# trukanduk/pq_huffman

Measured on AMD Instinct MI355X. Metric: Mvec/s encode+decode round-trip, 128-d fp32 M=8 K=256; % HBM-read roofline, higher is better.
Workload: dtype f32

## Files before the change

### include/pqh.h

```cpp
#ifndef _PQH_H
#define _PQH_H

#include <stddef.h>
#include <stdint.h>

#include "fast_nn_block.h"
#include "huffman.h"

#ifdef __cplusplus
extern "C" {
#endif

typedef enum {
    PQH_OK = 0,
    PQH_ERR_ARG = -1,
    PQH_ERR_NO_DEVICE = -2,
    PQH_ERR_HIP = -3,
    PQH_ERR_UNSUPPORTED = -4,
    PQH_ERR_CODE_TOO_LONG = -5,
    PQH_ERR_CORRUPT = -6,
    PQH_ERR_NOMEM = -7,
    PQH_ERR_CAPACITY = -8,
    PQH_ERR_REMOTE = -9,
    PQH_ERR_COMM = -10
} pqh_status_t;

typedef struct pqh_ctx pqh_ctx_t;

int pqh_ctx_create(pqh_ctx_t** ctx, int device);
int pqh_ctx_create_cu_limited(pqh_ctx_t** ctx, int device, int cus);
int pqh_ctx_create_cu_split(pqh_ctx_t** ctx, int device, int cus, int complement);
void* pqh_ctx_stream(const pqh_ctx_t* ctx);
int pqh_ctx_destroy(pqh_ctx_t* ctx);
int pqh_ctx_release_scratch(pqh_ctx_t* ctx);
int pqh_ctx_set_stream(pqh_ctx_t* ctx, void* hip_stream);
int pqh_ctx_sync(pqh_ctx_t* ctx);
enum { PQH_TUNE_ASSIGN_WGS_PER_CU = 1, PQH_TUNE_HIST_SPLIT = 2, PQH_TUNE_HIST_BLOCK = 3,
       PQH_TUNE_ENC_IMPL = 4, PQH_TUNE_SEARCH_GROUPS = 5 };
int pqh_ctx_set_tuning(pqh_ctx_t* ctx, int key, double value);
const char* pqh_status_string(int status);
const char* pqh_ctx_last_error(const pqh_ctx_t* ctx);
int pqh_device_count(int* count);

typedef struct pqh_pq pqh_pq_t;

int pqh_pq_create(pqh_ctx_t* ctx, const float* centroids, int m, int k, int dsub, pqh_pq_t** pq);
int pqh_pq_destroy(pqh_pq_t* pq);

int pqh_pq_assign(pqh_ctx_t* ctx, const pqh_pq_t* pq, const float* d_x, long long n,
                  long long ld_x, void* d_codes, uint32_t* d_counts, int mode);
int pqh_pq_assign_parts(pqh_ctx_t* ctx, const pqh_pq_t* pq, const float* d_x, long long n,
                        long long ld_x, void* d_codes, long long ld_codes, uint32_t* d_counts,
                        int mode);
int pqh_pq_last_rerank_count(pqh_ctx_t* ctx, unsigned long long* count);

int pqh_pq_error(pqh_ctx_t* ctx, const pqh_pq_t* pq, const float* d_x, long long n,
                 long long ld_x, const void* d_codes, double* error_out);
int pqh_pq_reconstruct(pqh_ctx_t* ctx, const pqh_pq_t* pq, const void* d_codes, long long n,
                       float* d_out, long long ld_out);

int pqh_kmeans_train(pqh_ctx_t* ctx, const float* d_x, long long n, long long ld_x, int m,
                     int k, int dsub, int iters, float* centroids);

int pqh_histogram(pqh_ctx_t* ctx, const void* d_codes, long long n, int m, int k, int context,
                  const void* d_prev_row, uint32_t* d_counts);
int pqh_histogram_set(pqh_ctx_t* ctx, const void* d_codes, long long n, int m, int k,
                      int context, const void* d_prev_row, uint32_t* d_counts);
long long pqh_histogram_partial_bytes(long long n, int m, int k);
int pqh_histogram_parts(pqh_ctx_t* ctx, const void* d_codes, long long ld_codes, long long n,
                        int m, int k, int context, const void* d_prev_row, uint32_t* d_counts,
                        int set);
// ... 294 lines not shown
```

### pq_huffman_amd/codec.py

```python
from __future__ import annotations

import ctypes
import os
import tempfile
from dataclasses import dataclass

import numpy as np

from .capi import (EncodeOptions, HuffmanCodebook, PqhError, check, lib)

_libc = ctypes.CDLL(None)
_libc.fopen.restype = ctypes.c_void_p
_libc.fopen.argtypes = [ctypes.c_char_p, ctypes.c_char_p]
_libc.fclose.argtypes = [ctypes.c_void_p]
_libc.fwrite.argtypes = [ctypes.c_void_p, ctypes.c_size_t, ctypes.c_size_t, ctypes.c_void_p]
_libc.fseek.argtypes = [ctypes.c_void_p, ctypes.c_long, ctypes.c_int]


def _ptr(t):
    if t is None:
        return None
    if isinstance(t, np.ndarray):
        return t.ctypes.data_as(ctypes.c_void_p)
    return ctypes.c_void_p(t.data_ptr())
# ... 4 lines not shown
    return torch


def device_count() -> int:
    n = ctypes.c_int(0)
    lib().pqh_device_count(ctypes.byref(n))
    return n.value


class Context:

    def __init__(self, device: int = 0, stream=None, cus: int = 0, complement: bool = False):
        torch = _torch()
        self._deps = 0
        self._closing = False
        self.device = device
        torch.cuda.set_device(device)
        self.ptr = ctypes.c_void_p()
        if cus != 0:
            check(lib().pqh_ctx_create_cu_split(ctypes.byref(self.ptr), device, cus,
                                                int(complement)), "pqh_ctx_create_cu_split")
            self.stream = torch.cuda.ExternalStream(lib().pqh_ctx_stream(self.ptr), device=device)
            return
        self.stream = stream or torch.cuda.current_stream(device)
        check(lib().pqh_ctx_create(ctypes.byref(self.ptr), device), "pqh_ctx_create")
        check(lib().pqh_ctx_set_stream(self.ptr, ctypes.c_void_p(self.stream.cuda_stream)),
              "pqh_ctx_set_stream")

    def set_stream(self, stream) -> None:
        self.stream = stream
        check(lib().pqh_ctx_set_stream(self.ptr, ctypes.c_void_p(stream.cuda_stream)))

    TUNE = {"assign_wgs_per_cu": 1, "hist_split": 2, "hist_block": 3, "enc_impl": 4,
            "search_groups": 5}

    def set_tuning(self, **kw) -> "Context":
        for key, value in kw.items():
            check(lib().pqh_ctx_set_tuning(self.ptr, self.TUNE[key], float(value)),
                  f"pqh_ctx_set_tuning({key})")
        return self

    def sync(self) -> None:
        check(lib().pqh_ctx_sync(self.ptr), "pqh_ctx_sync")

    def release_scratch(self) -> None:
        check(lib().pqh_ctx_release_scratch(self.ptr), "pqh_ctx_release_scratch")

    def last_error(self) -> str:
        return (lib().pqh_ctx_last_error(self.ptr) or b"").decode()

    def _retain(self) -> None:
        self._deps += 1

    def _release(self) -> None:
        self._deps -= 1
        if self._closing and self._deps <= 0:
            self.close()

    def close(self) -> None:
        if self._deps > 0:
            self._closing = True
            return
        if self.ptr:
            lib().pqh_ctx_destroy(self.ptr)
            self.ptr = ctypes.c_void_p()

    def __del__(self):
# ... 939 lines not shown
```

### pq_huffman_amd/csrc/hip/pqh_assign.hip

```cpp
#include <algorithm>
#include <cmath>
#include <cstdlib>
#include <cstring>
#include <type_traits>
#include <vector>

#include "pqh_internal.h"

typedef __bf16 bf16x8 __attribute__((ext_vector_type(8)));
typedef float f32x16 __attribute__((ext_vector_type(16)));
typedef float f32x4 __attribute__((ext_vector_type(4)));

namespace {

#ifndef PQH_ASSIGN_WPG
#define PQH_ASSIGN_WPG 4
#endif
#ifndef PQH_ASSIGN_OCC_LARGE
#define PQH_ASSIGN_OCC_LARGE 2
#endif
#ifndef PQH_ASSIGN_RING
#define PQH_ASSIGN_RING 4
#endif
#ifndef PQH_ASSIGN_NB
// ... 1 lines not shown
#endif
#ifndef PQH_ASSIGN_OCC
#define PQH_ASSIGN_OCC (PQH_ASSIGN_NB == 1 ? 4 : 3)
#endif
#ifndef PQH_ASSIGN_DEFER
#define PQH_ASSIGN_DEFER 1
#endif
#ifndef PQH_ASSIGN_RQ
#define PQH_ASSIGN_RQ 128
#endif
#ifndef PQH_ASSIGN_RRMASK
#define PQH_ASSIGN_RRMASK 1
#endif
#ifndef PQH_ASSIGN_RRPAIR
#define PQH_ASSIGN_RRPAIR 1
#endif
#ifndef PQH_ASSIGN_RRPACK
#define PQH_ASSIGN_RRPACK 1
#endif
#ifndef PQH_ASSIGN_RRPICK
#define PQH_ASSIGN_RRPICK 1
#endif
#ifndef PQH_ASSIGN_RRSKIP
#define PQH_ASSIGN_RRSKIP 1
#endif
#ifndef PQH_ASSIGN_HANDOVER
#define PQH_ASSIGN_HANDOVER 1
#endif
#ifndef PQH_ASSIGN_EARLYX
#define PQH_ASSIGN_EARLYX 1
#endif
constexpr int kRqLds = PQH_ASSIGN_RQ;
constexpr int kWavesPerWG = PQH_ASSIGN_WPG;
constexpr int kNB = PQH_ASSIGN_NB;
#ifndef PQH_ASSIGN_CLDS
#define PQH_ASSIGN_CLDS 0
#endif
#ifndef PQH_ASSIGN_SHAREA
#define PQH_ASSIGN_SHAREA 0
#endif
constexpr int kAG = 8;
#ifndef PQH_ASSIGN_XAUX
#define PQH_ASSIGN_XAUX 0
#endif
constexpr bool kCentLds = PQH_ASSIGN_CLDS != 0;

template <int D>
struct Plan {
    static constexpr int MAIN = 2 * D;
    static constexpr int PM = (MAIN + 15) / 16;
    static constexpr int PL = (D + 15) / 16;
    static constexpr int PA = PM;
};

#ifndef PQH_ASSIGN_ASMMIN
#define PQH_ASSIGN_ASMMIN 0
#endif
#if PQH_ASSIGN_ASMMIN
__device__ __forceinline__ unsigned med3u(unsigned a, unsigned b, unsigned c) {
    unsigned r;
    asm("v_med3_f32 %0, %1, %2, %3" : "=v"(r) : "v"(a), "v"(b), "v"(c));
    return r;
}

__device__ __forceinline__ unsigned min3d(unsigned a, unsigned b, unsigned c, unsigned after) {
    unsigned r;
// ... 99 lines not shown
    return 0.0f;
}

template <int D>
__device__ __forceinline__ float exact_dist(const float* x, const float* c) {
#pragma clang fp contract(off)
    float acc = 0.0f;
#pragma unroll
    for (int j = 0; j < D; ++j) {
        float d = __fsub_rn(x[j], c[j]);
        acc = __fadd_rn(acc, __fmul_rn(d, d));
    }
    return acc;
}

constexpr int kStampWaves = 8192;
__device__ unsigned long long g_assign_stamps[kStampWaves][4];
__device__ unsigned long long g_assign_rr[kStampWaves][4];
#ifdef PQH_ASSIGN_STAMPS
#define PQH_RR_STAMP(var)                                                \
    do {                                                                 \
        asm volatile("s_waitcnt vmcnt(0) lgkmcnt(0)" ::: "memory");      \
        var = __builtin_amdgcn_s_memrealtime();                          \
    } while (0)
#endif

template <int D>
struct Slice {
    static constexpr bool HALF = D % 16 == 0;
    static constexpr int NP = HALF ? D / 16 : 1;
    static constexpr int XD = HALF ? D / 2 : D;
    static __device__ __forceinline__ int dim(int j, int h) {
        return HALF ? 16 * (j >> 3) + 8 * h + (j & 7) : j;
    }
};

__device__ __forceinline__ unsigned partner32(unsigned v) {
    const auto sw = __builtin_amdgcn_permlane32_swap(v, v, false, false);
    return (threadIdx.x & 32) ? sw[0] : sw[1];
}

template <int D>
__device__ __forceinline__ float norm_part(const float* xs) {
    float X = 0.0f;
#pragma unroll
    for (int j = 0; j < Slice<D>::XD; ++j) X = fmaf(xs[j], xs[j], X);
    return X;
}

template <int D>
__device__ __forceinline__ float norm_x(const float* xs) {
    float X = norm_part<D>(xs);
    if constexpr (Slice<D>::HALF) {
        const auto sw = __builtin_amdgcn_permlane32_swap(__float_as_uint(X), __float_as_uint(X),
                                                         false, false);
        X = __uint_as_float(sw[0]) + __uint_as_float(sw[1]);
    }
    return X;
}

template <int D>
__device__ __forceinline__ bool has_lo(const float* xs) {
    constexpr int XD = Slice<D>::XD;
    unsigned o = __float_as_uint(xs[0]);
    int j = 1;
    for (; j + 1 < XD; j += 2)
// ... 177 lines not shown
}

template <int D, int KT>
__device__ __forceinline__ f32x16 tile_scores(const uint4* src, const float* Cn, int lane, int t,
                                              const bf16x8* Bm, const bf16x8* Bl, bool lo_pass) {
    using P = Plan<D>;
    bf16x8 a[P::PA];
#pragma unroll
    for (int p = 0; p < P::PA; ++p) a[p] = frag_at<KT>(src, p, t, lane);
    return tile_scores_a<D>(a, Bm, Bl, lo_pass, tile_norms(Cn, t, lane >> 5));
}

__device__ __forceinline__ int tile_row(int t, int i, int h) {
    return 32 * t + (i & 3) + 8 * (i >> 2) + 4 * h;
}

__device__ __forceinline__ uint32_t score_mask(const f32x16& acc, float thr, uint32_t bits) {
#if PQH_ASSIGN_RRMASK && defined(__HIP_DEVICE_COMPILE__)
#pragma unroll
    for (int i = 15; i >= 0; --i) {
        const unsigned long long le = __ballot(acc[i] <= thr);
        asm("v_addc_co_u32_e64 %0, vcc, %0, %0, %1" : "+v"(bits) : "s"(le) : "vcc");
    }
    return bits;
#else
    uint32_t mk = 0;
#pragma unroll
    for (int i = 0; i < 16; ++i) mk |= (acc[i] <= thr ? 1u : 0u) << i;
    return (bits << 16) | mk;
#endif
}

template <int D, int KT, typename CodeT>
__global__ void __launch_bounds__(64 * kWavesPerWG, D == 32 ? 2 : KT > 8 ? PQH_ASSIGN_OCC_LARGE : PQH_ASSIGN_OCC)
pq_assign_mfma(const float* __restrict__ x, long long n, long long ldx, int m_total,
               const bf16x8* __restrict__ afrag, const float* __restrict__ cnorm,
               const float* __restrict__ cent,
               const float* __restrict__ cmax, const float* __restrict__ sqrt_cmax,
               CodeT* __restrict__ codes, uint32_t* __restrict__ counts,
               unsigned long long* __restrict__ rerank, uint32_t* __restrict__ sched, int gx,
               unsigned long long* __restrict__ rerank_next, uint32_t* __restrict__ sched_next,
               int prio, long long ldc) {
    using P = Plan<D>;
    constexpr int K = KT * 32;
    constexpr bool kLdsA = KT <= 8;
    constexpr int PB = KT <= 8 ? 4 : 8;
    constexpr unsigned PMASK = (1u << PB) - 1;
    static_assert(2 * KT <= (1 << PB), "P-group index must fit the key's low bits");
    extern __shared__ uint32_t hist_dyn[];
    auto hist = [&](int w) -> uint32_t* { return hist_dyn + w * K; };
    __shared__ uint4 As[kLdsA ? P::PA * KT * 64 : 1];
    __shared__ __attribute__((aligned(64))) float Cn[KT * 2 * 16];
    __shared__ uint2 rqs[kWavesPerWG][kRqLds];
    constexpr int kPairs = PQH_ASSIGN_HANDOVER && kWavesPerWG % 2 == 0 ? kWavesPerWG / 2 : 0;
    __shared__ uint32_t rq_box[kPairs ? kPairs : 1];
#ifndef PQH_ASSIGN_XLDS
#define PQH_ASSIGN_XLDS 1
#endif
    constexpr bool kXLds = PQH_ASSIGN_XLDS && KT <= 8 && Slice<D>::XD % 4 == 0;
    __shared__ __attribute__((aligned(16))) float xst[kXLds ? kWavesPerWG : 1][kXLds ? kNB : 1]
                                                     [kXLds ? Slice<D>::XD / 4 : 1][kXLds ? 256 : 1];
    __shared__ __attribute__((aligned(16))) float Cf[kLdsA && kCentLds ? K * D : 1];
    constexpr bool kShareA = !kLdsA && PQH_ASSIGN_SHAREA != 0;
    constexpr int kAR = 2 * kAG;
    __shared__ __attribute__((aligned(16))) uint4 Ar[kShareA ? kAR * P::PA * 64 : 1];

    const int lane = threadIdx.x & 63;
    const int wave = __builtin_amdgcn_readfirstlane(threadIdx.x >> 6);
    const int L = blockIdx.x;
    const bool inter = (gx & 7) == 0;
    const int m = inter ? (L >> 3) % m_total : L / gx;
    const int bx = inter ? (L / (8 * m_total)) * 8 + (L & 7) : L % gx;
    const int r = lane & 31;
    const int h = lane >> 5;
    pqh_set_prio(prio);
    if (L == 0 && wave == 0) {
        if (sched_next)
            for (int q = lane; q < kSchedMax * kXcds; q += 64)
                __hip_atomic_store(sched_next + q * kSchedStride, 0u, __ATOMIC_RELAXED,
                                   __HIP_MEMORY_SCOPE_AGENT);
        if (lane == 0)
            __hip_atomic_store(rerank_next, 0ull, __ATOMIC_RELAXED, __HIP_MEMORY_SCOPE_AGENT);
    }
    constexpr bool kEarlyX = PQH_ASSIGN_EARLYX != 0 && !kShareA;
    auto fill_lds = [&]() {
        const uint4* src = reinterpret_cast<const uint4*>(afrag) + (long long)m * P::PA * KT * 64;
        constexpr int kNA = P::PA * KT * 64, kThreads = 64 * kWavesPerWG;
        if constexpr (kLdsA && kEarlyX && kNA % kThreads == 0 && KT * 2 * 16 <= kThreads) {
            const int tid = (int)threadIdx.x;
            if (KT * 2 * 16 == kThreads || tid < KT * 2 * 16)
                Cn[tid] = cnorm[(long long)m * KT * 2 * 16 + tid];
#pragma unroll
            for (int j = 0; j < kNA / kThreads; ++j) As[tid + j * kThreads] = src[tid + j * kThreads];
        } else {
            if constexpr (kLdsA)
                for (int i = threadIdx.x; i < kNA; i += blockDim.x) As[i] = src[i];
            for (int i = threadIdx.x; i < KT * 2 * 16; i += blockDim.x)
                Cn[i] = cnorm[(long long)m * KT * 2 * 16 + i];
        }
        if (kLdsA && counts)
            for (int i = lane; i < K; i += 64) hist(wave)[i] = 0;
        if constexpr (kLdsA && kCentLds)
            for (int i = threadIdx.x; i < K * D; i += blockDim.x) Cf[i] = cent[(long long)m * K * D + i];
        if ((int)threadIdx.x < kPairs) rq_box[threadIdx.x] = 0u;
        __syncthreads();
    };
    if constexpr (!kEarlyX) fill_lds();
    const uint4* const asrc =
        kLdsA ? As : reinterpret_cast<const uint4*>(afrag) + (long long)m * P::PA * KT * 64;
    const auto arsrc = __builtin_amdgcn_make_buffer_rsrc(
        const_cast<uint4*>(reinterpret_cast<const uint4*>(afrag) + (long long)m * P::PA * KT * 64),
        0, P::PA * KT * 64 * 16, 0x00020000);
#ifdef PQH_ASSIGN_STAMPS
    const unsigned long long st0 = __builtin_amdgcn_s_memtime();
    const unsigned long long rt0 = __builtin_amdgcn_s_memrealtime();
    unsigned long long nbdone = 0, rr_ticks = 0, rr_batches = 0;
    unsigned long long rr_x = 0, rr_scr = 0, rr_cand = 0, rr_rounds = 0;
#endif
    const float cm = cmax[m];
    const float sc = sqrt_cmax[m];
    const TauCoef tq = tau_coef(cm, sc, sqrt_cmax[m_total + m]);
    const float ninf = opaque_ninf();
    const unsigned keymask = PB == 4 ? ~PMASK : opaque_u32(~PMASK);
    const float* cl = kLdsA && kCentLds ? Cf : cent + (long long)m * K * D;
    const int n32 = (int)n;
    const int nblk = (n32 + 31) / 32;
    const int nfull = n32 / 32;
    unsigned long long slow_count = 0;

    constexpr bool HALF = Slice<D>::HALF;
    constexpr int XD = Slice<D>::XD;
// ... 17 lines not shown
            const unsigned last = (unsigned)(left < 31 ? left : 31);
            off = __umul24(min((unsigned)r, last), ldx4) + xh_off;
        }
        const float* xp = reinterpret_cast<const float*>(xm + row0 * (long long)ldx4 + off);
        if constexpr (XD % 4 == 0) {
#pragma unroll
            for (int j = 0; j < XD; j += 4) {
                const f32x4 q = *reinterpret_cast<const f32x4*>(xp + (HALF ? 16 * (j >> 3) + (j & 7) : j));
                dst[j] = q.x; dst[j + 1] = q.y; dst[j + 2] = q.z; dst[j + 3] = q.w;
            }
        } else {
#pragma unroll
            for (int j = 0; j < XD; ++j) dst[j] = xp[j];
        }
    };
    auto load_x_lds = [&](int b, int slot) {
#ifdef PQH_ASSIGN_NOMEM
        b &= 63;
#endif
        long long row0 = (long long)b * 32;
        unsigned off = xlane_off;
        if (b >= nfull) {
            row0 = row0 < n - 1 ? row0 : n - 1;
            const long long left = n - 1 - row0;
            const unsigned last = (unsigned)(left < 31 ? left : 31);
            off = __umul24(min((unsigned)r, last), ldx4) + xh_off;
        }
        const float* xp = reinterpret_cast<const float*>(xm + row0 * (long long)ldx4 + off);
#pragma unroll
        for (int j = 0; j < XD; j += 4) {
#if defined(__HIP_DEVICE_COMPILE__)
            __builtin_amdgcn_global_load_lds(
                xp + (HALF ? 16 * (j >> 3) + (j & 7) : j),
                (__attribute__((address_space(3))) void*)(&xst[wave][slot][j / 4][0]), 16, 0,
                PQH_ASSIGN_XAUX);
#else
            (void)xp;
#endif
        }
    };
    auto read_x_lds = [&](int slot, float* dst) {
#pragma unroll
        for (int j = 0; j < XD; j += 4) {
            const f32x4 q = *reinterpret_cast<const f32x4*>(&xst[wave][slot][j / 4][lane * 4]);
            dst[j] = q.x; dst[j + 1] = q.y; dst[j + 2] = q.z; dst[j + 3] = q.w;
        }
    };
    auto read_ring = [&](int t, bf16x8* a) {
#pragma unroll
        for (int p = 0; p < P::PA; ++p)
            a[p] = *reinterpret_cast<const bf16x8*>(&Ar[((t % kAR) * P::PA + p) * 64 + lane]);
    };
    auto dma_group = [&](int g) {
        if constexpr (kShareA) {
            const uint4* src = reinterpret_cast<const uint4*>(afrag) + (long long)m * P::PA * KT * 64;
            static_assert((kAG * P::PA) % kWavesPerWG == 0, "whole pieces per wave");
#pragma unroll
            for (int i = 0; i < (kAG * P::PA) / kWavesPerWG; ++i) {
                const int q = wave + i * kWavesPerWG;
                const int t = g * kAG + q / P::PA, p = q % P::PA;
#if defined(__HIP_DEVICE_COMPILE__)
                __builtin_amdgcn_global_load_lds(
                    src + (p * KT + t) * 64 + lane,
                    (__attribute__((address_space(3))) void*)(&Ar[((t % kAR) * P::PA + p) * 64]),
                    16, 0, 0);
#else
                (void)src; (void)t; (void)p;
#endif
            }
        }
    };
    unsigned qn = 0;

    auto body = [&](auto lo_c, long long blk0, float (*xs)[XD], const float* Xg,
                    const bool* any_lo) {
        constexpr bool LO = decltype(lo_c)::value;
        bf16x8 Bm[kNB][P::PM], Bl[kNB][P::PL];
// ... 206 lines not shown
        }
        constexpr int NG = (kNB + 1) / 2;
#pragma unroll
        for (int g = 0; g < NG; ++g) {
            const int ba = 2 * g, bb = 2 * g + 1 < kNB ? 2 * g + 1 : 2 * g;
            const bool pair = ba != bb;
            const auto s1 = __builtin_amdgcn_permlane32_swap(own1[ba], own1[bb], false, false);
            const auto s2 = __builtin_amdgcn_permlane32_swap(own2[ba], own2[bb], false, false);
            const auto sc = __builtin_amdgcn_permlane32_swap(cbits[ba], cbits[bb], false, false);
            const unsigned b1 = minu((unsigned)s1[0], (unsigned)s1[1]);
            const unsigned b2 = minu(minu((unsigned)s2[0], (unsigned)s2[1]),
                                     maxu((unsigned)s1[0], (unsigned)s1[1]));
            int code = (int)((unsigned)s1[0] == b1 ? (unsigned)sc[0] : (unsigned)sc[1]);
            const long long rowl = (blk0 + ba) * 32 + (pair ? lane : r);
            const bool valid = rowl < n;
            const bool own_lane = pair || h == 0;
            const float Xl = Xg[g];
            const bool finite = isfinite(Xl);
            const float tau = screen_tau(Xl, pair && h ? any_lo[bb] : any_lo[ba], tq);
            constexpr float kKeySlack = PB == 4 ? 0x1p-17f : 0x1p-13f;
            const float K1 = __uint_as_float(b1), K2 = __uint_as_float(b2);
            const float KA = max_abs(K1, K2);
            const bool slow = !(K2 - K1 > fmaf(kKeySlack, KA, tau)) || !finite;

            unsigned long long need = __ballot(slow && valid && own_lane);
            bool deferred = false;
            if (need) {
                slow_count += __popcll(need);
                const unsigned long long fin = need & __ballot(finite);
                const unsigned cnt = (unsigned)__popcll(fin);
                if (PQH_ASSIGN_DEFER && cnt && qn + cnt <= (unsigned)kRqLds) {
                    if (slow && valid && own_lane && finite) {
                        const float thr = fmaf(2.0f * kKeySlack, fabsf(K1), K1 + tau);
                        rqs[wave][qn + __builtin_amdgcn_mbcnt_hi((unsigned)(fin >> 32),
                                      __builtin_amdgcn_mbcnt_lo((unsigned)fin, 0u))] =
                            make_uint2((uint32_t)rowl, __float_as_uint(thr));
                    }
                    qn += cnt;
                    deferred = finite;
                    need &= ~fin;
                }
                unsigned long long todo = need;
                while (todo) {
                    const int rs = __ffsll((long long)todo) - 1;
                    todo &= todo - 1;
                    float xv[D];
                    const long long vrow = (blk0 + ba) * 32 + (pair ? rs : (rs & 31));
                    const float* xr = x + vrow * ldx + (long long)m * D;
#pragma unroll
                    for (int j = 0; j < D; ++j) xv[j] = xr[j];
                    float best = INFINITY;
                    int bidx = 0x7FFFFFFF;
#pragma unroll 1
                    for (int q = 0; q < K / 64; ++q) {
                        const int c = lane + 64 * q;
                        const float dd = exact_dist<D>(xv, cl + c * D);
                        if (dd < best) { best = dd; bidx = c; }
                    }
#pragma unroll
                    for (int off = 32; off >= 1; off >>= 1) {
                        const float ob = __shfl_xor(best, off);
                        const int oi = __shfl_xor(bidx, off);
                        if (ob < best || (ob == best && oi < bidx)) { best = ob; bidx = oi; }
                    }
                    if (lane == rs) code = bidx == 0x7FFFFFFF ? 0 : bidx;
                }
            }
// ... 16 lines not shown
        }
        return;
#endif
        constexpr int NG = (kNB + 1) / 2;
        float Xg[NG];
        bool any_lo[kNB];
        bool chunk_lo = false;
#pragma unroll
        for (int g = 0; g < NG; ++g) {
            const int ba = 2 * g, bb = 2 * g + 1 < kNB ? 2 * g + 1 : 2 * g;
            if (ba == bb) {
                Xg[g] = norm_x<D>(xs[ba]);
            } else if constexpr (Slice<D>::HALF) {
                const auto sw = __builtin_amdgcn_permlane32_swap(
                    __float_as_uint(norm_part<D>(xs[ba])), __float_as_uint(norm_part<D>(xs[bb])),
                    false, false);
                Xg[g] = __uint_as_float(sw[0]) + __uint_as_float(sw[1]);
            } else {
                const float xa_ = norm_x<D>(xs[ba]), xb_ = norm_x<D>(xs[bb]);
                Xg[g] = h ? xb_ : xa_;
            }
        }
#pragma unroll
        for (int b = 0; b < kNB; ++b) {
            any_lo[b] = __any(has_lo<D>(xs[b]));
            chunk_lo |= any_lo[b];
        }
        if (chunk_lo)
            body(std::true_type{}, blk0, xs, Xg, any_lo);
        else
            body(std::false_type{}, blk0, xs, Xg, any_lo);
    };

    const int wave_id = bx * kWavesPerWG + wave;
    const int waves_m = gx * kWavesPerWG;
    const int nchunk = (nblk + kNB - 1) / kNB;
    const int R = nchunk > waves_m ? (nchunk - waves_m + kXcds - 1) / kXcds : 0;
    uint32_t* head = sched && !kShareA ? sched + (long long)m * kXcds * kSchedStride : nullptr;
    int xr = head ? (int)(__builtin_amdgcn_s_getreg((3 << 11) | 20) & (kXcds - 1)) : 0;
    int tries = head && R > 0 ? 0 : kXcds;
    auto ticket = [&]() -> unsigned {
        unsigned t = __builtin_nondeterministic_value(0u);
        if (lane == 0)
            t = __hip_atomic_fetch_add(head + xr * kSchedStride, 1u, __ATOMIC_RELAXED,
                                       __HIP_MEMORY_SCOPE_AGENT);
        return t;
    };
    unsigned traw = 0;
    if (tries < kXcds) traw = ticket();
    auto next_dyn = [&]() -> int {
        while (tries < kXcds) {
            const int t = (int)__builtin_amdgcn_readfirstlane(traw);
            const int lo = waves_m + xr * R;
            if (t < std::min(R, nchunk - lo)) {
                traw = ticket();
                return lo + t;
            }
            if (++tries < kXcds) {
                xr = (xr + 1) & (kXcds - 1);
                traw = ticket();
            }
#ifdef PQH_ASSIGN_ENDPRIO
            __builtin_amdgcn_s_setprio(PQH_ASSIGN_ENDPRIO);
#endif
        }
        return -1;
    };
    auto rerank32 = [&](const uint2 ent, const bool valid) {
// ... 169 lines not shown
            const int code = bidx == 0x7FFFFFFF ? 0 : bidx;
            cbase[v * crs] = (CodeT)code;
            if (kLdsA && counts) atomicAdd(&hist(wave)[code], 1u);
        }
#ifdef PQH_ASSIGN_STAMPS
        rr_ticks += __builtin_amdgcn_s_memrealtime() - rr0;
        ++rr_batches;
#endif
    };
    if constexpr (kShareA) {
        const int nsuper = (nchunk + kWavesPerWG - 1) / kWavesPerWG;
        int sc = bx;
        dma_group(0);
        dma_group(1);
        asm volatile("s_waitcnt vmcnt(0)" ::: "memory");
        lds_barrier();
        int chs = sc * kWavesPerWG + wave;
        float xq[kNB][XD];
#pragma unroll
        for (int b = 0; b < kNB; ++b) load_x(chs * kNB + b, xq[b]);
        while (sc < nsuper) {
            float xa[kNB][XD];
#pragma unroll
            for (int b = 0; b < kNB; ++b)
#pragma unroll
                for (int j = 0; j < XD; ++j) xa[b][j] = xq[b][0 * j + j];
            const int nsc = sc + gx;
            const int nch = nsc * kWavesPerWG + wave;
            const int pre = nsc < nsuper ? nch : chs;
#pragma unroll
            for (int b = 0; b < kNB; ++b) load_x(pre * kNB + b, xq[b]);
            step((long long)chs * kNB, xa);
            while (qn >= 32u) {
                rerank32(rqs[wave][qn - 32u + (unsigned)r], true);
                qn -= 32u;
            }
            sc = nsc;
            chs = nch;
        }
        asm volatile("s_waitcnt vmcnt(0)" ::: "memory");
    }
    int ch = kShareA ? nchunk : wave_id;
    float xn[kXLds ? 1 : kNB][XD];
#pragma unroll
    for (int b = 0; b < kNB; ++b) {
        if constexpr (kXLds)
            load_x_lds(ch * kNB + b, b);
        else
            load_x(ch * kNB + b, xn[b]);
    }
    if constexpr (kEarlyX) fill_lds();
    while (ch < nchunk) {
        float xa[kNB][XD];
        if constexpr (kXLds) {
#pragma unroll
            for (int b = 0; b < kNB; ++b) read_x_lds(b, xa[b]);
            asm volatile("s_waitcnt lgkmcnt(0)" ::: "memory");
        } else {
#pragma unroll
            for (int b = 0; b < kNB; ++b)
#pragma unroll
                for (int j = 0; j < XD; ++j) xa[b][j] = xn[b][0 * j + j];
        }
        int nc;
        if (!head) {
            nc = ch + waves_m;
        } else {
            const int c = next_dyn();
            nc = c < 0 ? nchunk : c;
        }
        const int pre = nc < nchunk ? nc : ch;
#pragma unroll
        for (int b = 0; b < kNB; ++b) {
            if constexpr (kXLds)
                load_x_lds(pre * kNB + b, b);
            else
                load_x(pre * kNB + b, xn[b]);
        }
        step((long long)ch * kNB, xa);
        while (qn >= 32u) {
            rerank32(rqs[wave][qn - 32u + (unsigned)r], true);
            qn -= 32u;
        }
#ifdef PQH_ASSIGN_STAMPS
        nbdone += kNB;
#endif
        ch = nc;
    }
#ifdef PQH_ASSIGN_STAMPS
    const unsigned long long rt_loop = __builtin_amdgcn_s_memrealtime();
#endif
#ifdef PQH_ASSIGN_TAILPRIO
    __builtin_amdgcn_s_setprio(PQH_ASSIGN_TAILPRIO);
#endif
    if constexpr (kPairs > 0) {
        uint32_t got = 0u;
        if (lane == 0)
            got = __hip_atomic_exchange(&rq_box[wave >> 1], 0x80000000u | qn, __ATOMIC_ACQ_REL,
                                        __HIP_MEMORY_SCOPE_WORKGROUP);
        got = __builtin_amdgcn_readfirstlane(got);
        const unsigned pn = got & 0x7FFFFFFFu;
        if (got != 0u) {
            const unsigned tot = qn + pn;
#pragma unroll 1
            for (unsigned e0 = 0; e0 < tot; e0 += 32u) {
                const unsigned e = e0 + (unsigned)r;
                const bool valid = e < tot;
                const uint2 ent = !valid ? make_uint2(0u, 0u)
                                  : e < qn ? rqs[wave][e] : rqs[wave ^ 1][e - qn];
                rerank32(ent, valid);
            }
        }
    } else if (qn) {
        const bool valid = (unsigned)r < qn;
        rerank32(valid ? rqs[wave][r] : make_uint2(0u, 0u), valid);
    }
#ifdef PQH_ASSIGN_STAMPS
    {
        const unsigned gw = (unsigned)((m * gx + bx) * kWavesPerWG + wave);
        if (lane == 0 && gw < (unsigned)kStampWaves) {
            g_assign_rr[gw][0] = rr_x;
            g_assign_rr[gw][1] = rr_scr;
            g_assign_rr[gw][2] = rr_cand;
            g_assign_rr[gw][3] = rr_rounds;
            g_assign_stamps[gw][0] = rt0;
            g_assign_stamps[gw][1] = __builtin_amdgcn_s_memrealtime();
            g_assign_stamps[gw][2] = nbdone | ((__builtin_amdgcn_s_memtime() - st0) << 16);
            g_assign_stamps[gw][3] = (__builtin_amdgcn_s_getreg((3 << 11) | 20) & 15) |
                                     ((rt_loop - rt0) << 8) |
                                     (rr_ticks << 32) | (rr_batches << 56);
        }
    }
#endif
    if (kLdsA && counts) {
        __builtin_amdgcn_wave_barrier();
        for (int i = lane; i < K; i += 64) {
            uint32_t c = hist(wave)[i];
            if (c) atomicAdd(&counts[(long long)m * K + i], c);
        }
    }
    if (lane == 0 && slow_count) atomicAdd(rerank, slow_count);
}

template <typename CodeT>
__global__ void pq_assign_exact(const float* __restrict__ x, long long n, long long ldx, int m_total,
                                int k, int dsub, const float* __restrict__ cent,
                                CodeT* __restrict__ codes, uint32_t* __restrict__ counts,
                                long long ldc) {
#pragma clang fp contract(off)
    const long long gid = (long long)blockIdx.x * blockDim.x + threadIdx.x;
    if (gid >= n * m_total) return;
    const long long v = gid / m_total;
// ... 130 lines not shown
                        main[(size_t)row * slots + slot];
                }
    for (int t = 0; t < kt; ++t)
        for (int h = 0; h < 2; ++h)
            for (int i = 0; i < 16; ++i)
                cn[(size_t)m * kt * 32 + (t * 2 + h) * 16 + i] =
                    (float)norm[32 * t + (i & 3) + 8 * (i >> 2) + 4 * h];
}

template <int D>
int pa_of() { return Plan<D>::PA; }

int plan_pa(int dsub) {
    switch (dsub) {
        case 4: return pa_of<4>();
        case 6: return pa_of<6>();
        case 8: return pa_of<8>();
        case 12: return pa_of<12>();
        case 16: return pa_of<16>();
        case 32: return pa_of<32>();
        default: return 0;
    }
}

double assign_wgs_per_cu(const pqh_ctx* ctx, int occ) {
    double v = ctx->tune_wgs_per_cu;
    if (!(v > 0.0)) {
        const char* e = getenv("PQH_ASSIGN_WGS_PER_CU");
        v = e ? atof(e) : 0.0;
    }
    return v > 0.0 && v < occ ? v : (double)occ;
}

template <typename CodeT>
int launch_mfma(pqh_ctx* ctx, pqh_pq* pq, const float* x, long long n, long long ldx,
                CodeT* codes, uint32_t* counts, long long ldc) {
    const long long nblk = (n + 31) / 32;
    const int groups = pq->m;
    dim3 block(64 * kWavesPerWG);
    const int ring = (int)(ctx->assign_launches++ & 1);
    unsigned long long* rr = ctx->d_diag + (ring ? 4 : 0);
    unsigned long long* rr_next = ctx->d_diag + (ring ? 0 : 4);
    ctx->rerank_slot = ring ? 4 : 0;
#ifdef PQH_ASSIGN_STATIC
    uint32_t* sched = nullptr;
#else
    uint32_t* sched = pq->m <= kSchedMax ? ctx->d_sched + ring * kSchedSet : nullptr;
#endif
    const int prio = pqh_prio("ASSIGN", 0);
#define PQH_CASE(DD) PQH_CASE_KT(DD, 8)
#define PQH_CASE_KT(DD, KTT)                                                                \
    case DD: {                                                                              \
        int per_cu = 1;                                                                     \
        const size_t dyn = KTT <= 8 && counts ? (size_t)kWavesPerWG * 256 * 4 : 0;         \
        if (hipOccupancyMaxActiveBlocksPerMultiprocessor(                                   \
                &per_cu, (const void*)(pq_assign_mfma<DD, KTT, CodeT>), (int)block.x, dyn) != \
                hipSuccess || per_cu < 1)                                                   \
            per_cu = 1;                                                                     \
        long long gx = (long long)((double)ctx->num_cus * assign_wgs_per_cu(ctx, per_cu) / groups); \
        gx = std::max(1ll, std::min(gx, ((nblk + kNB - 1) / kNB + kWavesPerWG - 1) / kWavesPerWG)); \
        if (gx >= 16) gx &= ~7ll;      \
        hipLaunchKernelGGL((pq_assign_mfma<DD, KTT, CodeT>), dim3((unsigned)(gx * groups)), block, \
                           dyn, ctx->stream, x, n, ldx, pq->m, pq->d_afrag, pq->d_cn, pq->d_cent, \
                           pq->d_cmax, pq->d_sqc, codes, counts, rr, sched, (int)gx,         \
                           rr_next, sched ? ctx->d_sched + (1 - ring) * kSchedSet : nullptr, \
                           prio, ldc);                                                        \
        PQH_LAUNCH_CHECK(ctx);                                                              \
        break;                                                                              \
    }
    if (pq->k == 4096) {
        if constexpr (sizeof(CodeT) == 2) {
            switch (pq->dsub) {
                PQH_CASE_KT(16, 128)
                default: return PQH_ERR_UNSUPPORTED;
            }
        } else {
            return PQH_ERR_UNSUPPORTED;
        }
    } else if constexpr (sizeof(CodeT) == 1) {
        switch (pq->dsub) {
            PQH_CASE(4)
            PQH_CASE(6)
            PQH_CASE(8)
            PQH_CASE(12)
            PQH_CASE(16)
            PQH_CASE(32)
            default: return PQH_ERR_UNSUPPORTED;
        }
    } else {
        return PQH_ERR_UNSUPPORTED;
    }
#undef PQH_CASE
#undef PQH_CASE_KT
    PQH_LAUNCH_CHECK(ctx);
    return PQH_OK;
}

template <typename CodeT>
int launch_exact(pqh_ctx* ctx, pqh_pq* pq, const float* x, long long n, long long ldx,
                 CodeT* codes, uint32_t* counts, long long ldc) {
    const long long total = n * pq->m;
    if (total == 0) return PQH_OK;
    hipLaunchKernelGGL((pq_assign_exact<CodeT>), dim3((unsigned)((total + 255) / 256)), dim3(256),
                       0, ctx->stream, x, n, ldx, pq->m, pq->k, pq->dsub, pq->d_cent, codes,
                       counts, ldc);
    PQH_LAUNCH_CHECK(ctx);
    return PQH_OK;
}

}

extern "C" {

int pqh_pq_create(pqh_ctx_t* ctx, const float* centroids, int m, int k, int dsub, pqh_pq_t** out) {
    if (!ctx || !centroids || !out || m <= 0 || k <= 0 || dsub <= 0 || k > 65536)
        return PQH_ERR_ARG;
    int rc = pqh_use_device(ctx);
    if (rc) return rc;
    pqh_pq* pq = new pqh_pq();
    pq->ctx = ctx;
    pq->m = m;
    pq->k = k;
    pq->dsub = dsub;
    const size_t nc = (size_t)m * k * dsub;
    bool finite = true;
    for (size_t i = 0; i < nc; ++i) finite &= std::isfinite(centroids[i]);
    const int pa = plan_pa(dsub);
    pq->mfma_ok = finite && pa > 0 && (k == 256 || (k == 4096 && dsub == 16));
// ... 194 lines not shown
```

### pq_huffman_amd/csrc/hip/pqh_ctx.cpp

```cpp
#include <cstdlib>
#include <cstring>

#include <algorithm>
#include <vector>
#include <cmath>

#include "pqh_internal.h"

int pqh_set_error(pqh_ctx* ctx, int code, const char* fmt, ...) {
    if (ctx) {
        va_list ap;
        va_start(ap, fmt);
        vsnprintf(ctx->err, sizeof(ctx->err), fmt, ap);
        va_end(ap);
    }
    return code;
}

int pqh_kmeans_fixed_shift(float max_abs, long long n) {
    if (!(max_abs > 0.0f) || n <= 0) return 40;
    if (std::isinf(max_abs)) return -126;
    const double b = (double)max_abs * (double)n;
    int s = 61 - (int)std::ceil(std::log2(b));
    return std::max(-126, std::min(100, s));
// ... 157 lines not shown
    if (!ctx) return PQH_ERR_ARG;
    PQH_HIP(ctx, hipSetDevice(ctx->device));
    PQH_HIP(ctx, hipStreamSynchronize(ctx->stream));
    if (ctx->ws) (void)hipFree(ctx->ws);
    if (ctx->enc_scr) (void)hipFree(ctx->enc_scr);
    if (ctx->lb_state) (void)hipFree(ctx->lb_state);
    if (ctx->sort_state) (void)hipFree(ctx->sort_state);
    ctx->ws = ctx->enc_scr = nullptr;
    ctx->ws_bytes = ctx->enc_scr_bytes = 0;
    ctx->lb_state = nullptr;
    ctx->lb_cap = 0;
    ctx->sort_state = nullptr;
    ctx->sort_cap = 0;
    return PQH_OK;
}

int pqh_ctx_set_stream(pqh_ctx_t* ctx, void* hip_stream) {
    if (!ctx) return PQH_ERR_ARG;
    if (ctx->own_stream) {
        (void)hipStreamSynchronize(ctx->stream);
        (void)hipStreamDestroy(ctx->stream);
        ctx->own_stream = false;
    }
    ctx->stream = (hipStream_t)hip_stream;
    return PQH_OK;
}

int pqh_ctx_set_tuning(pqh_ctx_t* ctx, int key, double value) {
    if (!ctx || value < 0.0) return PQH_ERR_ARG;
    switch (key) {
        case PQH_TUNE_ASSIGN_WGS_PER_CU:
            ctx->tune_wgs_per_cu = value;
            return PQH_OK;
        case PQH_TUNE_HIST_SPLIT: {
            const int v = (int)value;
            if (v != 0 && v != 1 && v != 2 && v != 4 && v != 8) return PQH_ERR_ARG;
            ctx->tune_hist_split = v;
            return PQH_OK;
        }
        case PQH_TUNE_HIST_BLOCK: {
            const int v = (int)value;
            if (v != 0 && v != 256 && v != 1024) return PQH_ERR_ARG;
            ctx->tune_hist_block = v;
            return PQH_OK;
        }
        case PQH_TUNE_ENC_IMPL: {
            const int v = (int)value;
            if (v != 0 && v != 1 && v != 2) return PQH_ERR_ARG;
            ctx->tune_enc_impl = v;
            return PQH_OK;
        }
        case PQH_TUNE_SEARCH_GROUPS:
            if (value > 65535.0) return PQH_ERR_ARG;
            ctx->tune_search_groups = (int)value;
            return PQH_OK;
        default:
            return PQH_ERR_ARG;
    }
}

int pqh_ctx_sync(pqh_ctx_t* ctx) {
    if (!ctx) return PQH_ERR_ARG;
    PQH_HIP(ctx, hipStreamSynchronize(ctx->stream));
    return PQH_OK;
}

// ... 29 lines not shown
```

### pq_huffman_amd/csrc/hip/pqh_internal.h

```cpp
#pragma once

#include <hip/hip_runtime.h>

#include <cstdarg>
#include <cstdint>
#include <cstdio>

#include "pqh.h"

#if defined(__HIP_DEVICE_COMPILE__) && !defined(__gfx950__)
#error "pq_huffman_amd device code targets gfx950 only (--offload-arch=gfx950)"
#endif

struct pqh_tables;

struct pqh_ctx {
    int device = 0;
    int num_cus = 256;
    hipStream_t stream = nullptr;
    bool own_stream = false;
    char err[512] = {0};
    void* ws = nullptr;
    size_t ws_bytes = 0;
    unsigned long long* d_diag = nullptr;
    unsigned long long* lb_state = nullptr;
    long long lb_cap = 0;
    unsigned lb_epoch = 0;
    unsigned long long lb_ticket_base = 0;
    uint32_t* d_sched = nullptr;
    unsigned long long assign_launches = 0;
    unsigned long long* sort_state = nullptr;
    long long sort_cap = 0;
    unsigned sort_epoch = 0;
    unsigned long long sort_ticket_base = 0;
    int rerank_slot = 0;
    double tune_wgs_per_cu = 0.0;
    int tune_hist_split = 0;
    int tune_hist_block = 0;
    int tune_enc_impl = 0;
    int tune_search_groups = 0;
    void* enc_scr = nullptr;
    size_t enc_scr_bytes = 0;
};
constexpr int kDiagSlots = 16;
constexpr int kDiagIvf = 8;
constexpr int kSchedMax = 64;
constexpr int kXcds = 8;
constexpr int kSchedStride = 64;
constexpr long long kSchedSet = (long long)kSchedMax * kXcds * kSchedStride;

int pqh_set_error(pqh_ctx* ctx, int code, const char* fmt, ...);
int pqh_ensure_ws(pqh_ctx* ctx, size_t bytes);
int pqh_ensure_enc_scratch(pqh_ctx* ctx, size_t bytes);
int pqh_use_device(pqh_ctx* ctx);
int pqh_no_ctx_status();
int pqh_kmeans_fixed_shift(float max_abs, long long n);
int pqh_kmeans_absmax_launch(pqh_ctx* ctx, const float* d_x, long long n, long long ld_x, int d,
                             unsigned* d_max);
int pqh_kmeans_accum_launch(pqh_ctx* ctx, const float* d_x, long long n, long long ld_x, int m,
                            int k, int dsub, const void* d_codes, int s, long long* d_sums,
                            unsigned long long* d_cnt);
int pqh_kmeans_update_launch(pqh_ctx* ctx, const long long* d_sums, const unsigned long long* d_cnt,
                             long long cells, int dsub, int s, float* d_cent);
int pqh_pq_error_accum(pqh_ctx* ctx, const pqh_pq_t* pq, const float* d_x, long long n,
                       long long ld_x, const void* d_codes, double* sum);
int pqh_pq_view(const pqh_pq_t* pq, int* m, int* k, int* dsub, const float** d_cent);
extern "C" {
int pqh_histogram_set_dev(pqh_ctx_t* ctx, const void* d_codes, long long n, int m, int k,
                          const void* d_prev_row, const int* d_rawf, uint32_t* d_counts);
// ... 92 lines not shown
```

Baseline: 3272.

## Allow wider assign workgroups with per-wave dynamic LDS for x slices and rerank queues

Moves the per-wave x prefetch slices, rerank queues and histograms into one dynamic LDS region whose stride depends on the wave count. This lets the MFMA assign kernel launch with a variable number of waves per workgroup (up to 12), so more waves share one LDS copy of the centroid fragments. The wider form is only used when a tuning key or environment variable asks for it. The A-fragment fill is also rewritten as a batched vector load before the LDS stores. Raising launch bounds to 12 waves may cap registers per thread and hurt the default 4-wave path.

```diff
diff --git a/include/pqh.h b/include/pqh.h
--- a/include/pqh.h
+++ b/include/pqh.h
@@ -36,7 +36,7 @@
 int pqh_ctx_set_stream(pqh_ctx_t* ctx, void* hip_stream);
 int pqh_ctx_sync(pqh_ctx_t* ctx);
 enum { PQH_TUNE_ASSIGN_WGS_PER_CU = 1, PQH_TUNE_HIST_SPLIT = 2, PQH_TUNE_HIST_BLOCK = 3,
-       PQH_TUNE_ENC_IMPL = 4, PQH_TUNE_SEARCH_GROUPS = 5 };
+       PQH_TUNE_ENC_IMPL = 4, PQH_TUNE_SEARCH_GROUPS = 5, PQH_TUNE_ASSIGN_WAVES_PER_WG = 6 };
 int pqh_ctx_set_tuning(pqh_ctx_t* ctx, int key, double value);
 const char* pqh_status_string(int status);
 const char* pqh_ctx_last_error(const pqh_ctx_t* ctx);
diff --git a/pq_huffman_amd/codec.py b/pq_huffman_amd/codec.py
--- a/pq_huffman_amd/codec.py
+++ b/pq_huffman_amd/codec.py
@@ -60,7 +60,7 @@
         check(lib().pqh_ctx_set_stream(self.ptr, ctypes.c_void_p(stream.cuda_stream)))
 
     TUNE = {"assign_wgs_per_cu": 1, "hist_split": 2, "hist_block": 3, "enc_impl": 4,
-            "search_groups": 5}
+            "search_groups": 5, "assign_waves_per_wg": 6}
 
     def set_tuning(self, **kw) -> "Context":
         for key, value in kw.items():
diff --git a/pq_huffman_amd/csrc/hip/pqh_assign.hip b/pq_huffman_amd/csrc/hip/pqh_assign.hip
--- a/pq_huffman_amd/csrc/hip/pqh_assign.hip
+++ b/pq_huffman_amd/csrc/hip/pqh_assign.hip
@@ -57,6 +57,11 @@
 #endif
 constexpr int kRqLds = PQH_ASSIGN_RQ;
 constexpr int kWavesPerWG = PQH_ASSIGN_WPG;
+constexpr int kMaxWavesPerWG = 12;
+template <int D, int KT>
+constexpr int max_waves() {
+    return KT > 8 ? kWavesPerWG : std::max(kWavesPerWG, D == 32 ? 8 : kMaxWavesPerWG);
+}
 constexpr int kNB = PQH_ASSIGN_NB;
 #ifndef PQH_ASSIGN_CLDS
 #define PQH_ASSIGN_CLDS 0
@@ -222,6 +227,19 @@
     static constexpr int XD = HALF ? D / 2 : D;
     static __device__ __forceinline__ int dim(int j, int h) {
         return HALF ? 16 * (j >> 3) + 8 * h + (j & 7) : j;
+    }
+};
+
+#ifndef PQH_ASSIGN_XLDS
+#define PQH_ASSIGN_XLDS 1
+#endif
+template <int D, int KT>
+struct AssignLds {
+    static constexpr bool kXLds = PQH_ASSIGN_XLDS && KT <= 8 && Slice<D>::XD % 4 == 0;
+    static constexpr int kXstB = kXLds ? kNB * (Slice<D>::XD / 4) * 1024 : 0;
+    static constexpr int kRqB = kRqLds * 8;
+    static constexpr int wave_bytes(bool counts) {
+        return KT > 8 ? 0 : kXstB + kRqB + (counts ? KT * 32 * 4 : 0);
     }
 };
 
@@ -465,7 +483,7 @@
 }
 
 template <int D, int KT, typename CodeT>
-__global__ void __launch_bounds__(64 * kWavesPerWG, D == 32 ? 2 : KT > 8 ? PQH_ASSIGN_OCC_LARGE : PQH_ASSIGN_OCC)
+__global__ void __launch_bounds__((64 * max_waves<D, KT>()), D == 32 ? 2 : KT > 8 ? PQH_ASSIGN_OCC_LARGE : PQH_ASSIGN_OCC)
 pq_assign_mfma(const float* __restrict__ x, long long n, long long ldx, int m_total,
                const bf16x8* __restrict__ afrag, const float* __restrict__ cnorm,
                const float* __restrict__ cent,
@@ -480,19 +498,17 @@
     constexpr int PB = KT <= 8 ? 4 : 8;
     constexpr unsigned PMASK = (1u << PB) - 1;
     static_assert(2 * KT <= (1 << PB), "P-group index must fit the key's low bits");
-    extern __shared__ uint32_t hist_dyn[];
-    auto hist = [&](int w) -> uint32_t* { return hist_dyn + w * K; };
     __shared__ uint4 As[kLdsA ? P::PA * KT * 64 : 1];
     __shared__ __attribute__((aligned(64))) float Cn[KT * 2 * 16];
-    __shared__ uint2 rqs[kWavesPerWG][kRqLds];
-    constexpr int kPairs = PQH_ASSIGN_HANDOVER && kWavesPerWG % 2 == 0 ? kWavesPerWG / 2 : 0;
+    static_assert(kWavesPerWG % 2 == 0, "wave pairs (w, w ^ 1)");
+    constexpr int kPairs = PQH_ASSIGN_HANDOVER ? max_waves<D, KT>() / 2 : 0;
     __shared__ uint32_t rq_box[kPairs ? kPairs : 1];
-#ifndef PQH_ASSIGN_XLDS
-#define PQH_ASSIGN_XLDS 1
-#endif
     constexpr bool kXLds = PQH_ASSIGN_XLDS && KT <= 8 && Slice<D>::XD % 4 == 0;
-    __shared__ __attribute__((aligned(16))) float xst[kXLds ? kWavesPerWG : 1][kXLds ? kNB : 1]
-                                                     [kXLds ? Slice<D>::XD / 4 : 1][kXLds ? 256 : 1];
+    using Lds = AssignLds<D, KT>;
+    constexpr int kXstB = Lds::kXstB, kRqB = Lds::kRqB;
+    static_assert(!kXLds == !kXstB, "AssignLds sizes the x slices the kernel prefetches");
+    extern __shared__ __attribute__((aligned(16))) unsigned char dyn_lds[];
+    __shared__ uint2 rqs_static[kLdsA ? 1 : kWavesPerWG][kLdsA ? 1 : kRqLds];
     __shared__ __attribute__((aligned(16))) float Cf[kLdsA && kCentLds ? K * D : 1];
     constexpr bool kShareA = !kLdsA && PQH_ASSIGN_SHAREA != 0;
     constexpr int kAR = 2 * kAG;
@@ -500,6 +516,19 @@
 
     const int lane = threadIdx.x & 63;
     const int wave = __builtin_amdgcn_readfirstlane(threadIdx.x >> 6);
+    const int nw = kLdsA ? (int)(blockDim.x >> 6) : kWavesPerWG;
+    const int wstride = kXstB + kRqB + (counts ? K * 4 : 0);
+    auto rq_of = [&](int w) -> uint2* {
+        if constexpr (kLdsA)
+            return reinterpret_cast<uint2*>(dyn_lds + w * wstride + kXstB);
+        else
+            return rqs_static[w];
+    };
+    auto hist = [&](int w) -> uint32_t* {
+        return reinterpret_cast<uint32_t*>(dyn_lds + w * wstride + kXstB + kRqB);
+    };
+    float* const xst = reinterpret_cast<float*>(dyn_lds + wave * wstride);
+    uint2* const rqs = rq_of(wave);
     const int L = blockIdx.x;
     const bool inter = (gx & 7) == 0;
     const int m = inter ? (L >> 3) % m_total : L / gx;
@@ -518,18 +547,31 @@
     constexpr bool kEarlyX = PQH_ASSIGN_EARLYX != 0 && !kShareA;
     auto fill_lds = [&]() {
         const uint4* src = reinterpret_cast<const uint4*>(afrag) + (long long)m * P::PA * KT * 64;
-        constexpr int kNA = P::PA * KT * 64, kThreads = 64 * kWavesPerWG;
-        if constexpr (kLdsA && kEarlyX && kNA % kThreads == 0 && KT * 2 * 16 <= kThreads) {
-            const int tid = (int)threadIdx.x;
-            if (KT * 2 * 16 == kThreads || tid < KT * 2 * 16)
-                Cn[tid] = cnorm[(long long)m * KT * 2 * 16 + tid];
-#pragma unroll
-            for (int j = 0; j < kNA / kThreads; ++j) As[tid + j * kThreads] = src[tid + j * kThreads];
-        } else {
+        constexpr int kNA = P::PA * KT * 64;
+        auto fill_strided = [&]() {
             if constexpr (kLdsA)
                 for (int i = threadIdx.x; i < kNA; i += blockDim.x) As[i] = src[i];
             for (int i = threadIdx.x; i < KT * 2 * 16; i += blockDim.x)
                 Cn[i] = cnorm[(long long)m * KT * 2 * 16 + i];
+        };
+        if constexpr (kLdsA && kEarlyX && KT * 2 * 16 <= 64 * kWavesPerWG) {
+            const int tid = (int)threadIdx.x, nt = (int)blockDim.x;
+            constexpr int kNarrow = 64 * kWavesPerWG;
+            constexpr int kJ = (kNA + kNarrow - 1) / kNarrow;
+            typedef unsigned u32x4 __attribute__((ext_vector_type(4)));
+            const u32x4* const s4 = reinterpret_cast<const u32x4*>(src);
+            u32x4* const a4 = reinterpret_cast<u32x4*>(As);
+            u32x4 v[kJ];
+            float cn = 0.0f;
+            if (tid < KT * 2 * 16) cn = cnorm[(long long)m * KT * 2 * 16 + tid];
+#pragma unroll
+            for (int j = 0; j < kJ; ++j) v[j] = s4[min(tid + j * nt, kNA - 1)];
+            if (tid < KT * 2 * 16) Cn[tid] = cn;
+#pragma unroll
+            for (int j = 0; j < kJ; ++j)
+                if (tid + j * nt < kNA) a4[tid + j * nt] = v[j];
+        } else {
+            fill_strided();
         }
         if (kLdsA && counts)
             for (int i = lane; i < K; i += 64) hist(wave)[i] = 0;
@@ -613,7 +655,7 @@
 #if defined(__HIP_DEVICE_COMPILE__)
             __builtin_amdgcn_global_load_lds(
                 xp + (HALF ? 16 * (j >> 3) + (j & 7) : j),
-                (__attribute__((address_space(3))) void*)(&xst[wave][slot][j / 4][0]), 16, 0,
+                (__attribute__((address_space(3))) void*)(xst + (slot * (XD / 4) + j / 4) * 256), 16, 0,
                 PQH_ASSIGN_XAUX);
 #else
             (void)xp;
@@ -623,7 +665,8 @@
     auto read_x_lds = [&](int slot, float* dst) {
 #pragma unroll
         for (int j = 0; j < XD; j += 4) {
-            const f32x4 q = *reinterpret_cast<const f32x4*>(&xst[wave][slot][j / 4][lane * 4]);
+            const f32x4 q =
+                *reinterpret_cast<const f32x4*>(xst + (slot * (XD / 4) + j / 4) * 256 + lane * 4);
             dst[j] = q.x; dst[j + 1] = q.y; dst[j + 2] = q.z; dst[j + 3] = q.w;
         }
     };
@@ -896,7 +939,7 @@
                 if (PQH_ASSIGN_DEFER && cnt && qn + cnt <= (unsigned)kRqLds) {
                     if (slow && valid && own_lane && finite) {
                         const float thr = fmaf(2.0f * kKeySlack, fabsf(K1), K1 + tau);
-                        rqs[wave][qn + __builtin_amdgcn_mbcnt_hi((unsigned)(fin >> 32),
+                        rqs[qn + __builtin_amdgcn_mbcnt_hi((unsigned)(fin >> 32),
                                       __builtin_amdgcn_mbcnt_lo((unsigned)fin, 0u))] =
                             make_uint2((uint32_t)rowl, __float_as_uint(thr));
                     }
@@ -979,8 +1022,8 @@
             body(std::false_type{}, blk0, xs, Xg, any_lo);
     };
 
-    const int wave_id = bx * kWavesPerWG + wave;
-    const int waves_m = gx * kWavesPerWG;
+    const int wave_id = bx * nw + wave;
+    const int waves_m = gx * nw;
     const int nchunk = (nblk + kNB - 1) / kNB;
     const int R = nchunk > waves_m ? (nchunk - waves_m + kXcds - 1) / kXcds : 0;
     uint32_t* head = sched && !kShareA ? sched + (long long)m * kXcds * kSchedStride : nullptr;
@@ -1216,7 +1259,7 @@
             for (int b = 0; b < kNB; ++b) load_x(pre * kNB + b, xq[b]);
             step((long long)chs * kNB, xa);
             while (qn >= 32u) {
-                rerank32(rqs[wave][qn - 32u + (unsigned)r], true);
+                rerank32(rqs[qn - 32u + (unsigned)r], true);
                 qn -= 32u;
             }
             sc = nsc;
@@ -1263,7 +1306,7 @@
         }
         step((long long)ch * kNB, xa);
         while (qn >= 32u) {
-            rerank32(rqs[wave][qn - 32u + (unsigned)r], true);
+            rerank32(rqs[qn - 32u + (unsigned)r], true);
             qn -= 32u;
         }
 #ifdef PQH_ASSIGN_STAMPS
@@ -1291,17 +1334,17 @@
                 const unsigned e = e0 + (unsigned)r;
                 const bool valid = e < tot;
                 const uint2 ent = !valid ? make_uint2(0u, 0u)
-                                  : e < qn ? rqs[wave][e] : rqs[wave ^ 1][e - qn];
+                                  : e < qn ? rqs[e] : rq_of(wave ^ 1)[e - qn];
                 rerank32(ent, valid);
             }
         }
     } else if (qn) {
         const bool valid = (unsigned)r < qn;
-        rerank32(valid ? rqs[wave][r] : make_uint2(0u, 0u), valid);
+        rerank32(valid ? rqs[r] : make_uint2(0u, 0u), valid);
     }
 #ifdef PQH_ASSIGN_STAMPS
     {
-        const unsigned gw = (unsigned)((m * gx + bx) * kWavesPerWG + wave);
+        const unsigned gw = (unsigned)((m * gx + bx) * nw + wave);
         if (lane == 0 && gw < (unsigned)kStampWaves) {
             g_assign_rr[gw][0] = rr_x;
             g_assign_rr[gw][1] = rr_scr;
@@ -1498,42 +1541,90 @@
     return v > 0.0 && v < occ ? v : (double)occ;
 }
 
+int assign_waves_per_wg(const pqh_ctx* ctx) {
+    int v = ctx->tune_waves_per_wg;
+    if (v <= 0) {
+        const char* e = getenv("PQH_ASSIGN_WAVES_PER_WG");
+        v = e ? atoi(e) : 0;
+        if (v < 0 || v > kMaxWavesPerWG || (v & 1) || v == 2) v = 0;
+    }
+    return v;
+}
+
+struct AssignLaunch {
+    pqh_ctx* ctx;
+    pqh_pq* pq;
+    const float* x;
+    long long n, ldx, ldc;
+    uint32_t* counts;
+    unsigned long long *rr, *rr_next;
+    uint32_t *sched, *sched_next;
+    int prio;
+};
+
+template <int DD, int KTT, typename CodeT>
+int launch_form(const AssignLaunch& a, CodeT* codes) {
+    pqh_ctx* ctx = a.ctx;
+    using Lds = AssignLds<DD, KTT>;
+    const auto kern = pq_assign_mfma<DD, KTT, CodeT>;
+    const int groups = a.pq->m;
+    const long long nchunk = ((a.n + 31) / 32 + kNB - 1) / kNB;
+    const size_t wave_b = (size_t)Lds::wave_bytes(a.counts != nullptr);
+    int per_cu = 1;
+    if (hipOccupancyMaxActiveBlocksPerMultiprocessor(&per_cu, (const void*)kern, 64 * kWavesPerWG,
+                                                     kWavesPerWG * wave_b) != hipSuccess ||
+        per_cu < 1)
+        per_cu = 1;
+    const double tuned = assign_wgs_per_cu(ctx, per_cu);
+    int nw = kWavesPerWG;
+    long long gx = (long long)((double)ctx->num_cus * tuned / groups);
+    const long long gx_n = (nchunk + kWavesPerWG - 1) / kWavesPerWG;
+    if (KTT <= 8) {
+        const int forced = assign_waves_per_wg(ctx);
+        const int cap = std::min(max_waves<DD, KTT>(), kWavesPerWG * per_cu);
+        int wide = forced ? forced : kWavesPerWG;
+        wide = std::max(kWavesPerWG, std::min(wide, cap) & ~1);
+        if (wide != kWavesPerWG) {
+            nw = wide;
+            gx = std::min<long long>(ctx->num_cus / groups, (nchunk + nw - 1) / nw);
+        }
+    }
+    if (nw == kWavesPerWG) gx = std::min(gx, gx_n);
+    gx = std::max(1ll, gx);
+    if (gx >= 16) gx &= ~7ll;
+    const size_t dyn = (size_t)nw * wave_b;
+    const unsigned raise_bit = 1u << (DD & 31);
+    if (dyn > 48 * 1024 && !(ctx->assign_dyn_raised & raise_bit)) {
+        PQH_HIP(ctx, hipFuncSetAttribute((const void*)kern,
+                                         hipFuncAttributeMaxDynamicSharedMemorySize,
+                                         max_waves<DD, KTT>() * Lds::wave_bytes(true)));
+        ctx->assign_dyn_raised |= raise_bit;
+    }
+    hipLaunchKernelGGL(kern, dim3((unsigned)(gx * groups)), dim3(64 * nw), dyn, ctx->stream, a.x,
+                       a.n, a.ldx, a.pq->m, a.pq->d_afrag, a.pq->d_cn, a.pq->d_cent, a.pq->d_cmax,
+                       a.pq->d_sqc, codes, a.counts, a.rr, a.sched, (int)gx, a.rr_next,
+                       a.sched_next, a.prio, a.ldc);
+    PQH_LAUNCH_CHECK(ctx);
+    return PQH_OK;
+}
+
 template <typename CodeT>
 int launch_mfma(pqh_ctx* ctx, pqh_pq* pq, const float* x, long long n, long long ldx,
                 CodeT* codes, uint32_t* counts, long long ldc) {
-    const long long nblk = (n + 31) / 32;
-    const int groups = pq->m;
-    dim3 block(64 * kWavesPerWG);
     const int ring = (int)(ctx->assign_launches++ & 1);
-    unsigned long long* rr = ctx->d_diag + (ring ? 4 : 0);
-    unsigned long long* rr_next = ctx->d_diag + (ring ? 0 : 4);
     ctx->rerank_slot = ring ? 4 : 0;
 #ifdef PQH_ASSIGN_STATIC
     uint32_t* sched = nullptr;
 #else
     uint32_t* sched = pq->m <= kSchedMax ? ctx->d_sched + ring * kSchedSet : nullptr;
 #endif
-    const int prio = pqh_prio("ASSIGN", 0);
+    const AssignLaunch a{ctx, pq, x, n, ldx, ldc, counts,
+                         ctx->d_diag + (ring ? 4 : 0), ctx->d_diag + (ring ? 0 : 4), sched,
+                         sched ? ctx->d_sched + (1 - ring) * kSchedSet : nullptr,
+                         pqh_prio("ASSIGN", 0)};
 #define PQH_CASE(DD) PQH_CASE_KT(DD, 8)
-#define PQH_CASE_KT(DD, KTT)                                                                \
-    case DD: {                                                                              \
-        int per_cu = 1;                                                                     \
-        const size_t dyn = KTT <= 8 && counts ? (size_t)kWavesPerWG * 256 * 4 : 0;         \
-        if (hipOccupancyMaxActiveBlocksPerMultiprocessor(                                   \
-                &per_cu, (const void*)(pq_assign_mfma<DD, KTT, CodeT>), (int)block.x, dyn) != \
-                hipSuccess || per_cu < 1)                                                   \
-            per_cu = 1;                                                                     \
-        long long gx = (long long)((double)ctx->num_cus * assign_wgs_per_cu(ctx, per_cu) / groups); \
-        gx = std::max(1ll, std::min(gx, ((nblk + kNB - 1) / kNB + kWavesPerWG - 1) / kWavesPerWG)); \
-        if (gx >= 16) gx &= ~7ll;      \
-        hipLaunchKernelGGL((pq_assign_mfma<DD, KTT, CodeT>), dim3((unsigned)(gx * groups)), block, \
-                           dyn, ctx->stream, x, n, ldx, pq->m, pq->d_afrag, pq->d_cn, pq->d_cent, \
-                           pq->d_cmax, pq->d_sqc, codes, counts, rr, sched, (int)gx,         \
-                           rr_next, sched ? ctx->d_sched + (1 - ring) * kSchedSet : nullptr, \
-                           prio, ldc);                                                        \
-        PQH_LAUNCH_CHECK(ctx);                                                              \
-        break;                                                                              \
-    }
+#define PQH_CASE_KT(DD, KTT) \
+    case DD: return launch_form<DD, KTT, CodeT>(a, codes);
     if (pq->k == 4096) {
         if constexpr (sizeof(CodeT) == 2) {
             switch (pq->dsub) {
@@ -1558,8 +1649,6 @@
     }
 #undef PQH_CASE
 #undef PQH_CASE_KT
-    PQH_LAUNCH_CHECK(ctx);
-    return PQH_OK;
 }
 
 template <typename CodeT>
diff --git a/pq_huffman_amd/csrc/hip/pqh_ctx.cpp b/pq_huffman_amd/csrc/hip/pqh_ctx.cpp
--- a/pq_huffman_amd/csrc/hip/pqh_ctx.cpp
+++ b/pq_huffman_amd/csrc/hip/pqh_ctx.cpp
@@ -213,6 +213,12 @@
         case PQH_TUNE_ASSIGN_WGS_PER_CU:
             ctx->tune_wgs_per_cu = value;
             return PQH_OK;
+        case PQH_TUNE_ASSIGN_WAVES_PER_WG: {
+            const int v = (int)value;
+            if ((double)v != value || v > 12 || (v & 1) || v == 2) return PQH_ERR_ARG;
+            ctx->tune_waves_per_wg = v;
+            return PQH_OK;
+        }
         case PQH_TUNE_HIST_SPLIT: {
             const int v = (int)value;
             if (v != 0 && v != 1 && v != 2 && v != 4 && v != 8) return PQH_ERR_ARG;
diff --git a/pq_huffman_amd/csrc/hip/pqh_internal.h b/pq_huffman_amd/csrc/hip/pqh_internal.h
--- a/pq_huffman_amd/csrc/hip/pqh_internal.h
+++ b/pq_huffman_amd/csrc/hip/pqh_internal.h
@@ -35,6 +35,8 @@
     unsigned long long sort_ticket_base = 0;
     int rerank_slot = 0;
     double tune_wgs_per_cu = 0.0;
+    int tune_waves_per_wg = 0;
+    unsigned assign_dyn_raised = 0;
     int tune_hist_split = 0;
     int tune_hist_block = 0;
     int tune_enc_impl = 0;
```

Measured after the change: 3262. Within noise of the previous version (-0.3%).
